# google/uis-rnn

Measured on NVIDIA H100. Metric: predict_frames_per_sec_beam10_256d, higher is better.
Workload: dtype f32

## Files before the change

### uisrnn_b200/csrc/uis_prepass.cuh

```cuda
#pragma once
#include "uis_common.cuh"

namespace uis {

__global__ void cast_f64_f32_kernel(const double* __restrict__ in, float* __restrict__ out, size_t n) {
  size_t i = (size_t)blockIdx.x * blockDim.x + threadIdx.x;
  const size_t stride = (size_t)gridDim.x * blockDim.x;
  for (; i < n; i += stride) out[i] = __double2float_rn(in[i]);
}

__global__ void cast_pad_f64_f32_kernel(const double* __restrict__ in, float* __restrict__ out, size_t rows, int d, int dp) {
  size_t i = (size_t)blockIdx.x * blockDim.x + threadIdx.x;
  const size_t stride = (size_t)gridDim.x * blockDim.x, n = rows * (size_t)dp;
  for (; i < n; i += stride) {
    const size_t r = i / dp;
    const int c = (int)(i % dp);
    out[i] = c < d ? __double2float_rn(in[r * d + c]) : 0.f;
  }
}
__global__ void pad_rows_f32_kernel(const float* __restrict__ in, float* __restrict__ out, size_t rows, int d, int dp) {
  size_t i = (size_t)blockIdx.x * blockDim.x + threadIdx.x;
  const size_t stride = (size_t)gridDim.x * blockDim.x, n = rows * (size_t)dp;
  for (; i < n; i += stride) {
    const size_t r = i / dp;
    const int c = (int)(i % dp);
    out[i] = c < d ? in[r * d + c] : 0.f;
  }
}

constexpr int PBM = 128, PBN = 128, PBK = 16;
__global__ void __launch_bounds__(256) input_proj_kernel(const float* __restrict__ A, const float* __restrict__ Bt,
                                                         const float* __restrict__ bias, float* __restrict__ C,
                                                         int M, int N, int K) {
  __shared__ __align__(16) float As[PBK][PBM + 4];
  __shared__ __align__(16) float Bs[PBK][PBN];
  const int tid = threadIdx.x;
  const int m0 = blockIdx.y * PBM, n0 = blockIdx.x * PBN;
  const int tx = tid % 16, ty = tid / 16;
  float acc[8][8];
#pragma unroll
  for (int i = 0; i < 8; ++i)
#pragma unroll
    for (int q = 0; q < 8; ++q) acc[i][q] = 0.f;

  for (int k0 = 0; k0 < K; k0 += PBK) {
#pragma unroll
    for (int r = 0; r < 2; ++r) {
      const int f = tid + r * 256;
      const int row = f / 4, kq = (f % 4) * 4;
      float4 v = make_float4(0.f, 0.f, 0.f, 0.f);
      if (m0 + row < M && k0 + kq < K) v = *reinterpret_cast<const float4*>(A + (size_t)(m0 + row) * K + k0 + kq);
      As[kq + 0][row] = v.x; As[kq + 1][row] = v.y; As[kq + 2][row] = v.z; As[kq + 3][row] = v.w;
    }
#pragma unroll
    for (int r = 0; r < 2; ++r) {
      const int f = tid + r * 256;
      const int kk = f / 32, nq = (f % 32) * 4;
      float4 v = make_float4(0.f, 0.f, 0.f, 0.f);
      if (k0 + kk < K && n0 + nq < N) v = *reinterpret_cast<const float4*>(Bt + (size_t)(k0 + kk) * N + n0 + nq);
      *reinterpret_cast<float4*>(&Bs[kk][nq]) = v;
    }
    __syncthreads();
#pragma unroll
    for (int kk = 0; kk < PBK; ++kk) {
      const float4 a0 = *reinterpret_cast<const float4*>(&As[kk][ty * 8]);
      const float4 a1 = *reinterpret_cast<const float4*>(&As[kk][ty * 8 + 4]);
      const float4 b0 = *reinterpret_cast<const float4*>(&Bs[kk][tx * 4]);
      const float4 b1 = *reinterpret_cast<const float4*>(&Bs[kk][64 + tx * 4]);
      const float a[8] = {a0.x, a0.y, a0.z, a0.w, a1.x, a1.y, a1.z, a1.w};
      const float b[8] = {b0.x, b0.y, b0.z, b0.w, b1.x, b1.y, b1.z, b1.w};
#pragma unroll
      for (int i = 0; i < 8; ++i)
#pragma unroll
        for (int q = 0; q < 8; ++q) acc[i][q] = fmaf(a[i], b[q], acc[i][q]);
    }
    __syncthreads();
  }
#pragma unroll
  for (int i = 0; i < 8; ++i) {
    const int row = m0 + ty * 8 + i;
    if (row >= M) continue;
#pragma unroll
    for (int h = 0; h < 2; ++h) {
      const int coln = n0 + h * 64 + tx * 4;
      if (coln < N) {
        const float4 bv = *reinterpret_cast<const float4*>(bias + coln);
        float4 o;
        o.x = __fadd_rn(acc[i][h * 4 + 0], bv.x); o.y = __fadd_rn(acc[i][h * 4 + 1], bv.y);
        o.z = __fadd_rn(acc[i][h * 4 + 2], bv.z); o.w = __fadd_rn(acc[i][h * 4 + 3], bv.w);
        *reinterpret_cast<float4*>(C + (size_t)row * N + coln) = o;
      }
    }
  }
}

__global__ void __launch_bounds__(1024) init_state_kernel(const float* __restrict__ whh_t, const float* __restrict__ wih_up_t,
                                  const float* __restrict__ w1_t, const float* __restrict__ w2_t,
                                  const float* __restrict__ bih, const float* __restrict__ bhh,
                                  const float* __restrict__ b1, const float* __restrict__ b2,
                                  const float* __restrict__ h0, int H, int D, int depth, float* __restrict__ mean0,
                                  float* __restrict__ hidden0) {
  extern __shared__ float sm[];
  float* shp = sm; float* shx = sm + H; float* sa = sm + 2 * H;
  const int j = threadIdx.x;
  for (int l = 0; l < depth; ++l) {
    if (j < H) shp[j] = h0[(size_t)l * H + j];
    __syncthreads();
    float hn = 0.f;
    if (j < H) {
      const float* wh = whh_t + (size_t)l * H * 3 * H;
      float ar = 0.f, az = 0.f, an = 0.f;
      for (int k = 0; k < H; ++k) {
        const float x = shp[k];
        ar = fmaf(wh[(size_t)k * 3 * H + j], x, ar);
        az = fmaf(wh[(size_t)k * 3 * H + H + j], x, az);
        an = fmaf(wh[(size_t)k * 3 * H + 2 * H + j], x, an);
      }
      float ir = 0.f, iz = 0.f, in = 0.f;
      if (l > 0) {
        const float* wi = wih_up_t + (size_t)(l - 1) * H * 3 * H;
        for (int k = 0; k < H; ++k) {
          const float x = shx[k];
          ir = fmaf(wi[(size_t)k * 3 * H + j], x, ir);
          iz = fmaf(wi[(size_t)k * 3 * H + H + j], x, iz);
          in = fmaf(wi[(size_t)k * 3 * H + 2 * H + j], x, in);
        }
      }
      const float* bi = bih + (size_t)l * 3 * H;
      const float* bh = bhh + (size_t)l * 3 * H;
      const float r = sigmoid_f32(__fadd_rn(__fadd_rn(ir, bi[j]), __fadd_rn(ar, bh[j])));
      const float z = sigmoid_f32(__fadd_rn(__fadd_rn(iz, bi[H + j]), __fadd_rn(az, bh[H + j])));
      const float n = tanhf(__fadd_rn(__fadd_rn(in, bi[2 * H + j]), __fmul_rn(r, __fadd_rn(an, bh[2 * H + j]))));
      hn = __fadd_rn(__fmul_rn(__fsub_rn(shp[j], n), z), n);
      hidden0[(size_t)l * H + j] = hn;
    }
    __syncthreads();
    if (j < H) shx[j] = hn;
    __syncthreads();
  }
  if (j < H) {
    float a = 0.f;
    for (int k = 0; k < H; ++k) a = fmaf(w1_t[(size_t)k * H + j], shx[k], a);
    sa[j] = fmaxf(__fadd_rn(a, b1[j]), 0.f);
  }
  __syncthreads();
  if (j < D) {
    float a = 0.f;
    for (int k = 0; k < H; ++k) a = fmaf(w2_t[(size_t)k * D + j], sa[k], a);
    mean0[j] = __fadd_rn(a, b2[j]);
  }
}

}
```

### uisrnn_b200/csrc/uis_beam.cuh

```cuda
#pragma once
#include "uis_common.cuh"
#include "uis_beam_tc.cuh"
#include "uis_beam_stat.cuh"

namespace uis {

constexpr int kStages = 2;
constexpr int kStageBytes = 48 * 1024;
constexpr int kInitSlot = 0;
#ifndef UIS_CP_BEAM
#define UIS_CP_BEAM 20
#endif
constexpr int kCPBeam = UIS_CP_BEAM;
template <int H> struct BeamCP { static constexpr int value = H > 512 ? 8 : kCPBeam; };
template <int H> __host__ __device__ constexpr int beam_cp() { return BeamCP<H>::value; }
constexpr int kCPCluster = 12;
constexpr int kXchVals = 24;
constexpr int kCPTree = 16;
template <int H> struct TreeCP { static constexpr int value = H > 512 ? 8 : kCPTree; };
template <int H> __host__ __device__ constexpr int tree_cp() { return TreeCP<H>::value; }
constexpr int kMaxLanes = 8;
constexpr int kMaxBeam = 128;
constexpr int kMaxDepth = 4;

// ... 575 lines not shown
            pool_hidden_cta[(size_t)cc.lane[m0 + m] * lane_pool_h + (size_t)cc.dst[m0 + m] * DH + (size_t)l * H + j] = hnew;
        }
      }
    }
    named_bar_sync(1, NT);
#pragma unroll
    for (int u = 0; u < UPT; ++u)
#pragma unroll
      for (int c = 0; c < NC; ++c)
        reinterpret_cast<float4*>(XB + (size_t)(tid + NT * u) * C::CP)[c] =
            make_float4(hn_out[u][4 * c], hn_out[u][4 * c + 1], hn_out[u][4 * c + 2], hn_out[u][4 * c + 3]);
  }
  named_bar_sync(1, NT);
  if (tid == 0) { const long long now_ = clock64(); ph[2] += now_ - tmark; tmark = now_; }
  {
    float acc[C::R1][4 * NC];
    lin_pass<C, H, C::KT_1, C::KG1, C::R1, NC, true, XCL>(ring, full, empty, it, XB, acc, tid, lane, xrank, xsize);
    float out[UPT][4 * NC];
    ksplit_reduce<C, H, C::KG1, C::R1, UPT, NC>(acc, XA, out, tid);
    if constexpr (XCL) {
      static_assert(UPT * 4 * NC <= kXchVals, "cluster mode: W1 exchange in one round");
      float v[UPT * 4 * NC];
#pragma unroll
      for (int u = 0; u < UPT; ++u)
#pragma unroll
        for (int m = 0; m < 4 * NC; ++m) v[u * 4 * NC + m] = out[u][m];
      xch_allreduce<NT, UPT * 4 * NC>(*xc, v, tid);
#pragma unroll
      for (int u = 0; u < UPT; ++u)
#pragma unroll
        for (int m = 0; m < 4 * NC; ++m) out[u][m] = v[u * 4 * NC + m];
    }
#pragma unroll
    for (int u = 0; u < UPT; ++u)
#pragma unroll
      for (int c = 0; c < NC; ++c) {
        float4 v;
        v.x = fmaxf(__fadd_rn(out[u][4 * c + 0], b1r[u]), 0.f); v.y = fmaxf(__fadd_rn(out[u][4 * c + 1], b1r[u]), 0.f);
        v.z = fmaxf(__fadd_rn(out[u][4 * c + 2], b1r[u]), 0.f); v.w = fmaxf(__fadd_rn(out[u][4 * c + 3], b1r[u]), 0.f);
        reinterpret_cast<float4*>(XA + (size_t)(tid + NT * u) * C::CP)[c] = v;
      }
  }
  named_bar_sync(1, NT);
  if (tid == 0) { const long long now_ = clock64(); ph[3] += now_ - tmark; tmark = now_; }
  {
    float mu_old[4 * NC];
#pragma unroll
    for (int m = 0; m < 4 * NC; ++m)
      mu_old[m] = (m < Mp && tid < D)
                      ? pool_mean_cta[(size_t)cc.lane[m0 + m] * lane_pool_m + (size_t)cc.src[m0 + m] * D + tid]
                      : 0.f;
    float acc[C::R2][4 * NC];
    lin_pass<C, D, C::KT_2, C::KG2, C::R2, NC, true, XCL>(ring, full, empty, it, XA, acc, tid, lane, xrank, xsize);
    float out[1][4 * NC];
    ksplit_reduce<C, D, C::KG2, C::R2, 1, NC>(acc, XA, out, tid);
    if constexpr (XCL) xch_allreduce<NT, 4 * NC>(*xc, out[0], tid);
    if (tid < D) {
#pragma unroll
      for (int m = 0; m < 4 * NC; ++m) {
        if (m < Mp) {
          const float mval = __fadd_rn(out[0][m], b2r);
          const int n = cc.vis[m0 + m];
          const float mu = (n == 0) ? mval
                                    : __fdiv_rn(__fadd_rn(__fmul_rn(mu_old[m], (float)(n - 1)), mval), (float)n);
          pool_mean_cta[(size_t)cc.lane[m0 + m] * lane_pool_m + (size_t)cc.dst[m0 + m] * D + tid] = mu;
        }
      }
    }
  }
}

template <class C, bool DEEP, bool XCL = false>
__device__ __forceinline__ void run_pass_any(const BeamParams& p, const float* ring, uint64_t* full, uint64_t* empty,
                                             unsigned& it, float* XA, float* XB, const ColCtx cc, int m0, int Mp,
                                             float* pool_mean_cta, float* pool_hidden_cta, const float (&bh)[C::RG],
                                             const float (&b1r)[C::UPT], float b2r, int tid, int lane, long long* ph,
                                             long long& tmark, XchCtx* xc = nullptr) {
  const int nc = (Mp + 3) / 4;
#define UIS_RP(NCV, DEEPV) \
  run_pass<C, NCV, DEEPV, XCL>(p, ring, full, empty, it, XA, XB, cc, m0, Mp, pool_mean_cta, pool_hidden_cta, bh, b1r, b2r, tid, lane, ph, tmark, xc)
  if (nc == 1) UIS_RP(1, DEEP); else if (nc == 2) UIS_RP(2, DEEP); else if (nc == 3 || C::CP < 16) UIS_RP(3, DEEP);
  else if (nc == 4 || C::CP < 20) { if constexpr (C::CP >= 16) UIS_RP(4, DEEP); }
  else { if constexpr (C::CP >= 20) UIS_RP(5, DEEP); }
#undef UIS_RP
}

template <int H, int D, int CP, int NT>
__device__ __forceinline__ void stat_pass(const BeamParams& p, const float* sW, float* XA, float* XB, const ColCtx cc, int m0,
                                          int Mp, float* pool_mean_g, float* pool_hidden_g, float* scratch_g, unsigned* bar,
                                          unsigned& epoch, int q, int tid, long long* ph, long long& tmark) {
  using S = StatCfg<H, D>;
  const size_t lane_pool_h = (size_t)p.P * H, lane_pool_m = (size_t)p.P * D;
  stat_dot<H, S::R0, CP, NT>(sW, S::LD, 0, XA, XB, Mp, tid);
  named_bar_sync(1, NT);
  if (tid < S::UG * CP) {
    const int m = tid % CP, u = tid / CP, j = q * S::UG + u;
    if (m < Mp) {
      const float ar = stat_sum<S::R0, CP, NT>(XB, 0 * S::UG + u, m);
      const float az = stat_sum<S::R0, CP, NT>(XB, 1 * S::UG + u, m);
      const float an = stat_sum<S::R0, CP, NT>(XB, 2 * S::UG + u, m);
      const float* gi = p.gi + (size_t)cc.girow[m0 + m] * 3 * H;
      const float r = sigmoid_f32(__fadd_rn(gi[j], __fadd_rn(ar, __ldg(p.bhh + j))));
      const float z = sigmoid_f32(__fadd_rn(gi[H + j], __fadd_rn(az, __ldg(p.bhh + H + j))));
      const float n = tanhf(__fadd_rn(gi[2 * H + j], __fmul_rn(r, __fadd_rn(an, __ldg(p.bhh + 2 * H + j)))));
      const float ho = XA[(size_t)j * CP + m];
      pool_hidden_g[(size_t)cc.lane[m0 + m] * lane_pool_h + (size_t)cc.dst[m0 + m] * H + j] =
          __fadd_rn(__fmul_rn(__fsub_rn(ho, n), z), n);
    }
  }
  stat_group_sync<NT>(bar, epoch, tid);
  if (tid == 0) { const long long now_ = clock64(); ph[2] += now_ - tmark; tmark = now_; }
  for (int i = tid; i < Mp * H; i += NT) {
    const int m = i / H, k = i % H;
    XA[(size_t)k * CP + m] = __ldcg(pool_hidden_g + (size_t)cc.lane[m0 + m] * lane_pool_h + (size_t)cc.dst[m0 + m] * H + k);
  }
  named_bar_sync(1, NT);
  stat_dot<H, S::R1, CP, NT>(sW, S::LD, S::R0, XA, XB, Mp, tid);
  named_bar_sync(1, NT);
  if (tid < S::R1 * CP) {
    const int m = tid % CP, u = tid / CP, j = q * S::R1 + u;
    if (m < Mp)
      scratch_g[(size_t)m * H + j] = fmaxf(__fadd_rn(stat_sum<S::R1, CP, NT>(XB, u, m), __ldg(p.b1 + j)), 0.f);
  }
  stat_group_sync<NT>(bar, epoch, tid);
  if (tid == 0) { const long long now_ = clock64(); ph[3] += now_ - tmark; tmark = now_; }
  for (int i = tid; i < Mp * H; i += NT) {
    const int m = i / H, k = i % H;
    XA[(size_t)k * CP + m] = __ldcg(scratch_g + (size_t)m * H + k);
  }
  named_bar_sync(1, NT);
  stat_dot<H, S::R2, CP, NT>(sW, S::LD, S::R0 + S::R1, XA, XB, Mp, tid);
  named_bar_sync(1, NT);
  if (tid < S::R2 * CP) {
    const int m = tid % CP, u = tid / CP, d = q * S::R2 + u;
    if (m < Mp) {
      const float mval = __fadd_rn(stat_sum<S::R2, CP, NT>(XB, u, m), __ldg(p.b2 + d));
      const int n = cc.vis[m0 + m];
      const float mu_old = __ldcg(pool_mean_g + (size_t)cc.lane[m0 + m] * lane_pool_m + (size_t)cc.src[m0 + m] * D + d);
      const float mu = (n == 0) ? mval : __fdiv_rn(__fadd_rn(__fmul_rn(mu_old, (float)(n - 1)), mval), (float)n);
      pool_mean_g[(size_t)cc.lane[m0 + m] * lane_pool_m + (size_t)cc.dst[m0 + m] * D + d] = mu;
    }
  }
  stat_group_sync<NT>(bar, epoch, tid);
}

template <int H, int D, int N, class Idle>
__device__ __forceinline__ void tc_run_pass(const BeamParams& p, const unsigned char* ring, unsigned char* bop,
                                            const TcBars& tb, unsigned& tbox, const ColCtx cc, int m0, int Mp,
                                            float* pool_mean_cta, float* pool_hidden_cta, float* scratch_cta, int tid,
                                            int lane, int warp, long long* ph, long long& tmark, long long* tstat,
                                            Idle idle_work) {
  using TC = TcCfg<H, D, N>;
  constexpr int NT = 256, NI = N / 8;
  constexpr int KB = (NI == 6) ? 2 : 4, WB = (NI == 6) ? 3 : NI;
  auto hslot = [&](int g, int s) { return pool_hidden_cta + (size_t)(g * p.P + s) * H; };
  auto mslot = [&](int g, int s) { return pool_mean_cta + (size_t)(g * p.P + s) * D; };
  const int wg = warp >> 2;
  const int r0 = wg * 64 + (warp & 3) * 16 + (lane >> 2);
  const int cq = 2 * (lane & 3);
  long long* ts = (tid == 0) ? tstat : nullptr;
  const long long t_in = clock64();
  float acc[TC::NACC];
  auto stage_b = [&](auto src, float scale) {
    const long long w0 = clock64();
    tc_gather_b<H, N, NT>(bop, src, Mp, scale, tid);
    tc_publish_b<NT>();
    if (ts) ts[2] += clock64() - w0;
  };
  if (tid < Mp && (tid == 0 || cc.lane[m0 + tid] != cc.lane[m0 + tid - 1]))
    prefetch_l2_bulk(p.gi + (size_t)cc.girow[m0 + tid] * 3 * H, 3 * H * 4);
  stage_b([&](int m) -> const float* {
    return hslot(cc.lane[m0 + m], cc.src[m0 + m]); }, p.tc_sh);
  if (tid == 0) { const long long now_ = clock64(); ph[1] += now_ - tmark; tmark = now_; }
  idle_work();
  if (tid == 0) { const long long now_ = clock64(); ph[7] += now_ - tmark; tmark = now_; }
  static_assert(H >= NT, "gate parking: 2 * (N / 2) * NT floats within the [N][H] scratch");
  float* park = scratch_cta + tid;
  for (int ut = 0; ut < TC::UT; ++ut) {
    const int j0 = ut * 128 + r0;
    {
      float v[TC::NV];
#pragma unroll
      for (int g = 0; g < 2; ++g) {
        tc_tile<TC>(acc, ring, bop, tb, tbox, wg, lane, ts);
        tc_fold<TC>(acc, v, p.tc_inv_hh);
        const float bh[2] = {__ldg(p.bhh + g * H + j0), __ldg(p.bhh + g * H + j0 + 8)};
#pragma unroll
        for (int q = 0; q < TC::NV; ++q) park[(g * TC::NV + q) * NT] = __fadd_rn(v[q], bh[(q >> 1) & 1]);
      }
    }
    tc_tile<TC>(acc, ring, bop, tb, tbox, wg, lane, ts);
    float an[TC::NV];
    tc_fold<TC>(acc, an, p.tc_inv_hh);
    {
      const float bh[2] = {__ldg(p.bhh + 2 * H + j0), __ldg(p.bhh + 2 * H + j0 + 8)};
#pragma unroll
      for (int q = 0; q < TC::NV; ++q) an[q] = __fadd_rn(an[q], bh[(q >> 1) & 1]);
    }
#pragma unroll
    for (int k0 = 0; k0 < 2 * NI; k0 += KB) {
      float gr[KB][2], gz[KB][2], gn[KB][2], pr[KB][2], pz[KB][2], ho[KB][2];
#pragma unroll
      for (int b = 0; b < KB; ++b) {
        const int i = (k0 + b) >> 1, e = (k0 + b) & 1, m = 8 * i + cq + e;
        if (m < Mp) {
          const float* gi = p.gi + (size_t)cc.girow[m0 + m] * 3 * H + j0;
          const float* hs = hslot(cc.lane[m0 + m], cc.src[m0 + m]) + j0;
#pragma unroll
          for (int h = 0; h < 2; ++h) {
            const int v = 4 * i + 2 * h + e;
            gr[b][h] = __ldg(gi + 8 * h); gz[b][h] = __ldg(gi + H + 8 * h); gn[b][h] = __ldg(gi + 2 * H + 8 * h);
            pr[b][h] = park[v * NT]; pz[b][h] = park[(TC::NV + v) * NT];
            ho[b][h] = hs[8 * h];
          }
        }
      }
#pragma unroll
      for (int b = 0; b < KB; ++b) {
        const int i = (k0 + b) >> 1, e = (k0 + b) & 1, m = 8 * i + cq + e;
        if (m < Mp) {
          float* hd = hslot(cc.lane[m0 + m], cc.dst[m0 + m]) + j0;
#pragma unroll
          for (int h = 0; h < 2; ++h) {
            const int v = 4 * i + 2 * h + e;
            const float rg = sigmoid_f32(__fadd_rn(gr[b][h], pr[b][h]));
            const float zg = sigmoid_f32(__fadd_rn(gz[b][h], pz[b][h]));
            const float ng = tanhf(__fadd_rn(gn[b][h], __fmul_rn(rg, an[v])));
            hd[8 * h] = __fadd_rn(__fmul_rn(__fsub_rn(ho[b][h], ng), zg), ng);
          }
        }
      }
    }
  }
  named_bar_sync(1, NT);
  if (tid == 0) { const long long now_ = clock64(); ph[2] += now_ - tmark; tmark = now_; }
  stage_b([&](int m) -> const float* {
    return hslot(cc.lane[m0 + m], cc.dst[m0 + m]); }, p.tc_sh);
  for (int mt = 0; mt < TC::T2; ++mt) {
    float v1[TC::NV];
    tc_tile<TC>(acc, ring, bop, tb, tbox, wg, lane, ts);
    tc_fold<TC>(acc, v1, p.tc_inv_1);
#pragma unroll
    for (int h = 0; h < 2; ++h) {
      const int j = mt * 128 + r0 + 8 * h;
      const float b1j = __ldg(p.b1 + j);
#pragma unroll
      for (int i = 0; i < NI; ++i)
#pragma unroll
        for (int e = 0; e < 2; ++e) {
          const int m = 8 * i + cq + e;
          if (m < Mp) scratch_cta[(size_t)m * H + j] = fmaxf(__fadd_rn(v1[4 * i + 2 * h + e], b1j), 0.f);
        }
    }
  }
  named_bar_sync(1, NT);
  if (tid == 0) { const long long now_ = clock64(); ph[3] += now_ - tmark; tmark = now_; }
  stage_b([&](int m) -> const float* { return scratch_cta + (size_t)m * H; }, p.tc_sa);
  for (int mt = 0; mt < TC::T3; ++mt) {
    float v2[TC::NV];
    tc_tile<TC>(acc, ring, bop, tb, tbox, wg, lane, ts);
    tc_fold<TC>(acc, v2, p.tc_inv_2);
#pragma unroll
    for (int h = 0; h < 2; ++h) {
      const int d = mt * 128 + r0 + 8 * h;
      const float b2d = __ldg(p.b2 + d);
#pragma unroll
      for (int i0 = 0; i0 < NI; i0 += WB) {
        float mu_old[WB][2];
#pragma unroll
        for (int b = 0; b < WB; ++b)
#pragma unroll
          for (int e = 0; e < 2; ++e) {
            const int m = 8 * (i0 + b) + cq + e;
            if (m < Mp) mu_old[b][e] = mslot(cc.lane[m0 + m], cc.src[m0 + m])[d];
          }
#pragma unroll
        for (int b = 0; b < WB; ++b)
#pragma unroll
          for (int e = 0; e < 2; ++e) {
            const int m = 8 * (i0 + b) + cq + e;
            if (m < Mp) {
              const float mval = __fadd_rn(v2[4 * (i0 + b) + 2 * h + e], b2d);
              const int n = cc.vis[m0 + m];
              const float mu = (n == 0) ? mval : __fdiv_rn(__fadd_rn(__fmul_rn(mu_old[b][e], (float)(n - 1)), mval), (float)n);
              mslot(cc.lane[m0 + m], cc.dst[m0 + m])[d] = mu;
            }
          }
      }
    }
  }
  if (ts) ts[3] += clock64() - t_in;
}

template <int H, int D, bool DEEP, int XM = 0, int TCN = 0>
__global__ void __launch_bounds__(Cfg<H, D>::BLOCK, 1) uis_beam_kernel(const __grid_constant__ BeamParams p) {
  constexpr bool XCL = XM == 1, STAT = XM == 2;
  using C = Cfg<H, D, (XCL || STAT) ? kCPCluster : BeamCP<H>::value>;
  constexpr int NT = C::NT, NW = C::NW, UPT = C::UPT;
  constexpr bool TC = TCN > 0;
  static_assert(!TC || (!DEEP && !XCL && !STAT && NT == 256 && C::REBALANCE), "tensor-core pass: depth 1, one CTA per lane group");
  static_assert(!STAT || (!DEEP && NT == 256), "stationary-weights mode: depth 1, 256 consumer threads");
  using TCC = TcCfg<TC ? H : 512, TC ? D : 256, TC ? TCN : 48>;
  extern __shared__ __align__(128) unsigned char smem_raw[];
  unsigned char* smem = TC ? reinterpret_cast<unsigned char*>((reinterpret_cast<uintptr_t>(smem_raw) + 1023) & ~(uintptr_t)1023)
                           : smem_raw;
  const int B = p.B, Kcap = p.Kcap, G = p.G;
  const SmemLayout L_ = make_layout<H, D, C::CP, XCL, TCN, STAT>(B, Kcap, G);
  const SmemLayout& L = TC ? p.tc_layout : L_;
  if constexpr (TC)
    if (p.tc_layout.total == 0) __trap();
  const int sq = STAT ? (int)(blockIdx.x % kStatGroup) : 0, sgroup = STAT ? (int)(blockIdx.x / kStatGroup) : 0;
  float* ring = reinterpret_cast<float*>(smem + L.ring);
  float* XA = reinterpret_cast<float*>(smem + L.xa);
  float* XB = reinterpret_cast<float*>(smem + L.xb);
  float* wv = reinterpret_cast<float*>(smem + L.wv);
  int* colarr = reinterpret_cast<int*>(smem + L.cols);
  uint64_t* full = reinterpret_cast<uint64_t*>(smem + L.bars);
  uint64_t* empty = full + (TC ? TCC::STAGES : kStages);
  volatile int* misc = reinterpret_cast<volatile int*>(smem + L.misc);
  TcBars tb{full, empty};

  const int tid = threadIdx.x, lane = tid & 31, warp = tid >> 5;

  if (tid == 0) {
    if constexpr (TC) {
      for (int s = 0; s < TCC::STAGES; ++s) {
        mbar_init(&tb.full[s], 1);
        mbar_init(&tb.empty[s], NW);
      }
    } else {
      for (int s = 0; s < kStages; ++s) {
        mbar_init(&full[s], 1);
        mbar_init(&empty[s], NW);
      }
    }
    for (int i = 0; i < 16; ++i) misc[i] = 0;
    if constexpr (TC)
      for (int i = 16; i < 20; ++i) reinterpret_cast<long long*>(smem + L.phase)[i] = 0;
    if constexpr (XCL) {
      uint64_t* xbar = reinterpret_cast<uint64_t*>(smem + L.xbar);
      mbar_init(&xbar[0], cluster_nctarank() - 1);
      mbar_init(&xbar[1], cluster_nctarank() - 1);
      misc[MI_QNEXT] = (int)cluster_id_x();
    }
    if constexpr (STAT) misc[MI_QNEXT] = sgroup;
    fence_mbar_init();
  }
  __syncthreads();
  if constexpr (XCL) cluster_sync_all();

  if (warp >= NW) {
    if constexpr (STAT) return;
    if constexpr (TC) asm volatile("setmaxnreg.dec.sync.aligned.u32 40;");
    else if constexpr (C::REBALANCE) asm volatile("setmaxnreg.dec.sync.aligned.u32 24;");
    if constexpr (TC) {
      if (warp == NW) tc_producer_loop<TCC, H>(&p.tc_wmap, reinterpret_cast<unsigned char*>(ring), tb, &misc[MI_DONE]);
    } else {
      if (warp == NW && lane == 0) producer_loop<C, XCL>(p, ring, full, empty, misc);
    }
    return;
  }
  if constexpr (TC) asm volatile("setmaxnreg.inc.sync.aligned.u32 232;");
  else if constexpr (C::REBALANCE && !STAT) asm volatile("setmaxnreg.inc.sync.aligned.u32 240;");

  auto lane_base = [&](int g) -> unsigned char* { return smem + L.lanes + (size_t)g * L.lane_stride; };
  auto LSp = [&](int g) -> volatile int* { return reinterpret_cast<volatile int*>(lane_base(g) + L.l_ls); };
  const int DH = p.depth * H;
  const size_t pool_m_stride = (size_t)p.P * D, pool_h_stride = (size_t)p.P * DH;
  float* pool_mean_cta = p.pool_mean + (size_t)(STAT ? sgroup : blockIdx.x) * G * pool_m_stride;
  float* pool_hidden_cta = p.pool_hidden + (size_t)(STAT ? sgroup : blockIdx.x) * G * pool_h_stride;
  unsigned* bp_cta = p.bp + (size_t)blockIdx.x * G * p.maxN * B;
  const unsigned PW = (unsigned)(p.P + 31) / 32;
  const float INF = __int_as_float(0x7f800000);
  const int bbits = B > 32 ? 7 : 5;

  float bh[C::RG], b1r[UPT];
#pragma unroll
  for (int i = 0; i < C::RG; ++i) bh[i] = TC ? 0.f : p.bhh[(i / UPT) * H + tid + NT * (i % UPT)];
#pragma unroll
  for (int u = 0; u < UPT; ++u) b1r[u] = TC ? 0.f : p.b1[tid + NT * u];
  const float b2r = (tid < D && !TC) ? p.b2[tid] : 0.f;
// ... 617 lines not shown
```

### uisrnn_b200/csrc/uis_beam_tc.cuh

```cuda
#pragma once
#include <cuda.h>
#include <cuda_fp16.h>
#include "uis_common.cuh"

namespace uis {

constexpr int kTcBoxBytes = 16384;

template <int H, int D, int N>
struct TcCfg {
  static constexpr int KA = H / 64;
  static constexpr int UT = H / 128;
  static constexpr int T1 = 3 * UT, T2 = H / 128, T3 = D / 128;
  static constexpr int TILES = T1 + T2 + T3;
  static constexpr int ROWS = 3 * H + H + D;
  static constexpr int NP = 2 * N;
  static constexpr int NACC = NP / 2;
  static constexpr int NV = N / 2;
  static constexpr int ATOM_BYTES = NP * 128;
  static constexpr int BOP_BYTES = KA * ATOM_BYTES;
  static constexpr int STAGES = (N <= 32) ? 8 : 4;
  static_assert(H % 128 == 0 && D % 128 == 0, "tensor-core pass: 128-row tiles");
  static_assert(NP == 64 || NP == 96, "wgmma instantiations: N = 32 or 48 columns");
};

__device__ __forceinline__ uint64_t tc_desc_sw128(uint32_t saddr) {
  uint64_t d = 0;
  d |= (uint64_t)((saddr >> 4) & 0x3fff);
  d |= (uint64_t)1 << 16;
  d |= (uint64_t)(1024 >> 4) << 32;
  d |= (uint64_t)1 << 62;
  return d;
}
__device__ __forceinline__ void wgmma_fence() { asm volatile("wgmma.fence.sync.aligned;" ::: "memory"); }
__device__ __forceinline__ void wgmma_commit() { asm volatile("wgmma.commit_group.sync.aligned;" ::: "memory"); }
template <int PENDING>
__device__ __forceinline__ void wgmma_wait() { asm volatile("wgmma.wait_group.sync.aligned %0;" ::"n"(PENDING) : "memory"); }

template <int NP> struct Wgmma;
template <> struct Wgmma<96> {
  static __device__ __forceinline__ void mma(float (&d)[48], uint64_t adesc, uint64_t bdesc, uint32_t acc) {
    asm volatile(
        "{\n\t.reg .pred p;\n\tsetp.ne.b32 p, %50, 0;\n\t"
        "wgmma.mma_async.sync.aligned.m64n96k16.f32.f16.f16 {%0, %1, %2, %3, %4, %5, %6, %7, %8, %9, %10, %11, %12, %13, %14, %15, %16, %17, %18, %19, %20, %21, %22, %23, %24, %25, %26, %27, %28, %29, %30, %31, %32, %33, %34, %35, %36, %37, %38, %39, %40, %41, %42, %43, %44, %45, %46, %47}, %48, %49, p, 1, 1, 0, 0;\n\t}"
        : "+f"(d[0]), "+f"(d[1]), "+f"(d[2]), "+f"(d[3]), "+f"(d[4]), "+f"(d[5]), "+f"(d[6]), "+f"(d[7]), "+f"(d[8]), "+f"(d[9]), "+f"(d[10]), "+f"(d[11]), "+f"(d[12]), "+f"(d[13]), "+f"(d[14]), "+f"(d[15]), "+f"(d[16]), "+f"(d[17]), "+f"(d[18]), "+f"(d[19]), "+f"(d[20]), "+f"(d[21]), "+f"(d[22]), "+f"(d[23]), "+f"(d[24]), "+f"(d[25]), "+f"(d[26]), "+f"(d[27]), "+f"(d[28]), "+f"(d[29]), "+f"(d[30]), "+f"(d[31]), "+f"(d[32]), "+f"(d[33]), "+f"(d[34]), "+f"(d[35]), "+f"(d[36]), "+f"(d[37]), "+f"(d[38]), "+f"(d[39]), "+f"(d[40]), "+f"(d[41]), "+f"(d[42]), "+f"(d[43]), "+f"(d[44]), "+f"(d[45]), "+f"(d[46]), "+f"(d[47])
        : "l"(adesc), "l"(bdesc), "r"(acc)
        : "memory");
  }
};
template <> struct Wgmma<64> {
  static __device__ __forceinline__ void mma(float (&d)[32], uint64_t adesc, uint64_t bdesc, uint32_t acc) {
    asm volatile(
        "{\n\t.reg .pred p;\n\tsetp.ne.b32 p, %34, 0;\n\t"
        "wgmma.mma_async.sync.aligned.m64n64k16.f32.f16.f16 {%0, %1, %2, %3, %4, %5, %6, %7, %8, %9, %10, %11, %12, %13, %14, %15, %16, %17, %18, %19, %20, %21, %22, %23, %24, %25, %26, %27, %28, %29, %30, %31}, %32, %33, p, 1, 1, 0, 0;\n\t}"
        : "+f"(d[0]), "+f"(d[1]), "+f"(d[2]), "+f"(d[3]), "+f"(d[4]), "+f"(d[5]), "+f"(d[6]), "+f"(d[7]), "+f"(d[8]), "+f"(d[9]), "+f"(d[10]), "+f"(d[11]), "+f"(d[12]), "+f"(d[13]), "+f"(d[14]), "+f"(d[15]), "+f"(d[16]), "+f"(d[17]), "+f"(d[18]), "+f"(d[19]), "+f"(d[20]), "+f"(d[21]), "+f"(d[22]), "+f"(d[23]), "+f"(d[24]), "+f"(d[25]), "+f"(d[26]), "+f"(d[27]), "+f"(d[28]), "+f"(d[29]), "+f"(d[30]), "+f"(d[31])
        : "l"(adesc), "l"(bdesc), "r"(acc)
        : "memory");
  }
};

__device__ __forceinline__ void tc_tma_load_2d(void* dst, const CUtensorMap* map, int c0, int c1, uint64_t* bar) {
  asm volatile(
      "cp.async.bulk.tensor.2d.shared::cluster.global.mbarrier::complete_tx::bytes [%0], [%1, {%3, %4}], [%2];" ::"r"(
          smem_u32(dst)),
      "l"(reinterpret_cast<uint64_t>(map)), "r"(smem_u32(bar)), "r"(c0), "r"(c1)
      : "memory");
}

__device__ __forceinline__ void tc_mbar_wait(uint64_t* bar, uint32_t parity) {
  if (mbar_try_wait(bar, parity)) return;
  const long long t0 = clock64();
  unsigned spins = 0;
  while (!mbar_try_wait(bar, parity)) {
    if ((++spins & 0x3ffu) == 0 && clock64() - t0 > 8000000000ll) __trap();
  }
}

__device__ __forceinline__ bool tc_wait_or_done(uint64_t* bar, uint32_t parity, volatile int* done_flag) {
  for (;;) {
    uint32_t ok;
    asm volatile(
        "{\n\t.reg .pred p;\n\t"
        "mbarrier.try_wait.parity.shared::cta.b64 p, [%1], %2, %3;\n\t"
        "selp.u32 %0, 1, 0, p;\n\t}"
        : "=r"(ok)
        : "r"(smem_u32(bar)), "r"(parity), "r"(4000u)
        : "memory");
    if (ok) return true;
    if (*done_flag) return false;
  }
}

__device__ __forceinline__ bool tc_elect_one() {
  uint32_t pred;
  asm volatile("{\n\t.reg .pred p;\n\telect.sync _|p, 0xffffffff;\n\tselp.u32 %0, 1, 0, p;\n\t}" : "=r"(pred));
  return pred != 0;
}

struct TcBars {
  uint64_t* full;
  uint64_t* empty;
};

template <class TC, int H>
__device__ __forceinline__ int tc_tile_row0(int t) {
  if (t < TC::T1) return (t % 3) * H + (t / 3) * 128;
  return 3 * H + (t - TC::T1) * 128;
}

template <class TC, int H>
__device__ void tc_producer_loop(const CUtensorMap* wmap, unsigned char* ring, const TcBars& b, volatile int* done_flag) {
  unsigned it = 0;
  bool run = true;
  while (run) {
    for (int t = 0; t < TC::TILES && run; ++t) {
      const int row0 = tc_tile_row0<TC, H>(t);
      for (int pl = 0; pl < 2 && run; ++pl) {
        for (int ka = 0; ka < TC::KA; ++ka, ++it) {
          const unsigned s = it % TC::STAGES, ph = (it / TC::STAGES) & 1;
          if (!tc_wait_or_done(&b.empty[s], ph ^ 1, done_flag)) { run = false; break; }
          if (tc_elect_one()) {
            mbar_arrive_expect_tx(&b.full[s], kTcBoxBytes);
            tc_tma_load_2d(ring + (size_t)s * kTcBoxBytes, wmap, ka * 64, pl * TC::ROWS + row0, &b.full[s]);
          }
          __syncwarp();
        }
      }
    }
  }
  for (unsigned j = (it > (unsigned)TC::STAGES) ? it - TC::STAGES : 0; j < it; ++j)
    tc_mbar_wait(&b.full[j % TC::STAGES], (j / TC::STAGES) & 1);
}

template <class TC>
__device__ __forceinline__ void tc_tile(float (&acc)[TC::NACC], const unsigned char* ring, const unsigned char* bop,
                                        const TcBars& b, unsigned& box, int wg, int lane, long long* tstat) {
  const uint64_t desc0 = tc_desc_sw128(0);
  const uint32_t a16 = (smem_u32(ring) + (uint32_t)wg * (kTcBoxBytes / 2)) >> 4, b16 = smem_u32(bop) >> 4;
#pragma unroll
  for (int i = 0; i < TC::NACC; ++i) acc[i] = 0.f;
  unsigned prev = 0;
#pragma unroll 1
  for (int q = 0; q < 2 * TC::KA; ++q, ++box) {
    const unsigned s = box % TC::STAGES, par = (box / TC::STAGES) & 1u;
    if (!mbar_try_wait(&b.full[s], par)) {
      const long long w0 = tstat ? clock64() : 0;
      tc_mbar_wait(&b.full[s], par);
      if (tstat) tstat[0] += clock64() - w0;
    }
    const uint64_t adesc = desc0 + (uint64_t)(a16 + s * (kTcBoxBytes >> 4));
    const uint64_t bdesc = desc0 + (uint64_t)(b16 + (uint32_t)(q % TC::KA) * (TC::ATOM_BYTES >> 4));
    wgmma_fence();
#pragma unroll
    for (int kk = 0; kk < 4; ++kk) Wgmma<TC::NP>::mma(acc, adesc + 2 * kk, bdesc + 2 * kk, (q | kk) != 0);
    wgmma_commit();
    if (q > 0) {
      wgmma_wait<1>();
      __syncwarp();
      if (lane == 0) mbar_arrive(&b.empty[prev]);
    }
    prev = s;
  }
  const long long w0 = tstat ? clock64() : 0;
  wgmma_wait<0>();
  if (tstat) tstat[1] += clock64() - w0;
  __syncwarp();
  if (lane == 0) mbar_arrive(&b.empty[prev]);
}

template <class TC>
__device__ __forceinline__ void tc_fold(const float (&acc)[TC::NACC], float (&v)[TC::NV], float inv) {
  constexpr int LO = TC::NACC / 2;
#pragma unroll
  for (int i = 0; i < TC::NV; ++i) v[i] = __fmul_rn(__fmaf_rn(acc[LO + i], 0x1p-11f, acc[i]), inv);
}

template <int H, int N, int NTHREADS, class SrcFn>
__device__ __forceinline__ void tc_gather_b(unsigned char* bop, SrcFn src, int Mp, float scale, int tid) {
  constexpr int PPC = H / 2;
  constexpr int CG = NTHREADS / PPC;
  static_assert(NTHREADS % PPC == 0 && CG >= 1, "gather mapping");
  const int pair = tid % PPC, cg = tid / PPC;
  const int k = 2 * pair;
  const uint32_t koff = (uint32_t)(k >> 6) * (2u * N * 128u) + (uint32_t)(k & 7) * 2u;
  const uint32_t kchunk = (uint32_t)(k & 63) >> 3;
  constexpr int UNR = 8;
  for (int m0 = cg; m0 < Mp; m0 += CG * UNR) {
    float2 v[UNR];
#pragma unroll
    for (int u = 0; u < UNR; ++u) {
      const int m = m0 + u * CG;
      v[u] = (m < Mp) ? *reinterpret_cast<const float2*>(src(m) + k) : make_float2(0.f, 0.f);
    }
#pragma unroll
    for (int u = 0; u < UNR; ++u) {
      const int m = m0 + u * CG;
      if (m < Mp) {
        const float x0 = v[u].x * scale, x1 = v[u].y * scale;
        const __half h0 = __float2half_rn(x0), h1 = __float2half_rn(x1);
        const __half l0 = __float2half_rn((x0 - __half2float(h0)) * 2048.f);
        const __half l1 = __float2half_rn((x1 - __half2float(h1)) * 2048.f);
        const uint32_t off = koff + (uint32_t)m * 128u + ((kchunk ^ ((uint32_t)m & 7u)) << 4);
        *reinterpret_cast<__half2*>(bop + off) = __halves2half2(h0, h1);
        *reinterpret_cast<__half2*>(bop + off + (uint32_t)N * 128u) = __halves2half2(l0, l1);
      }
    }
  }
}
template <int NTHREADS>
__device__ __forceinline__ void tc_publish_b() {
  fence_proxy_async();
  named_bar_sync(1, NTHREADS);
}

}
```

Measured before the change: 2.175 million.

## Double-buffer input projection GEMM tiles with cp.async prefetch

Converts the input projection GEMM to double-buffered shared memory. The next K-tile of A goes through registers and the next tile of B is fetched with cp.async, both overlapped with the FMA loop on the current tile. This removes one __syncthreads per iteration and hides global load latency. It also adds launch_bounds minBlocks=2, which caps registers and doubles shared memory use and could cause spills. The input projection is a prepass, so its share of end-to-end beam-search frames/sec is likely small.

New measurement: 2.190 million (median of 6 runs). No clear change (+0.7%).

```diff
diff --git a/uisrnn_b200/csrc/uis_prepass.cuh b/uisrnn_b200/csrc/uis_prepass.cuh
--- a/uisrnn_b200/csrc/uis_prepass.cuh
+++ b/uisrnn_b200/csrc/uis_prepass.cuh
@@ -29,44 +29,57 @@
 }
 
 constexpr int PBM = 128, PBN = 128, PBK = 16;
-__global__ void __launch_bounds__(256) input_proj_kernel(const float* __restrict__ A, const float* __restrict__ Bt,
-                                                         const float* __restrict__ bias, float* __restrict__ C,
-                                                         int M, int N, int K) {
-  __shared__ __align__(16) float As[PBK][PBM + 4];
-  __shared__ __align__(16) float Bs[PBK][PBN];
+__global__ void __launch_bounds__(256, 2) input_proj_kernel(const float* __restrict__ A, const float* __restrict__ Bt,
+                                                            const float* __restrict__ bias, float* __restrict__ C,
+                                                            int M, int N, int K) {
+  __shared__ __align__(16) float As[2][PBK][PBM + 4];
+  __shared__ __align__(16) float Bs[2][PBK][PBN];
   const int tid = threadIdx.x;
   const int m0 = blockIdx.y * PBM, n0 = blockIdx.x * PBN;
   const int tx = tid % 16, ty = tid / 16;
+  float4 ra[2];
+  auto load = [&](int k0, int s) {
+#pragma unroll
+    for (int r = 0; r < 2; ++r) {
+      const int f = tid + r * 256;
+      const int row = f / 4, kq = (f % 4) * 4;
+      ra[r] = make_float4(0.f, 0.f, 0.f, 0.f);
+      if (m0 + row < M && k0 + kq < K) ra[r] = *reinterpret_cast<const float4*>(A + (size_t)(m0 + row) * K + k0 + kq);
+      const int kk = f / 32, nq = (f % 32) * 4;
+      float* bs = &Bs[s][kk][nq];
+      if (k0 + kk < K && n0 + nq < N) cp_async16(bs, Bt + (size_t)(k0 + kk) * N + n0 + nq);
+      else *reinterpret_cast<float4*>(bs) = make_float4(0.f, 0.f, 0.f, 0.f);
+    }
+    cp_async_commit();
+  };
+  auto store = [&](int s) {
+#pragma unroll
+    for (int r = 0; r < 2; ++r) {
+      const int f = tid + r * 256;
+      const int row = f / 4, kq = (f % 4) * 4;
+      As[s][kq + 0][row] = ra[r].x; As[s][kq + 1][row] = ra[r].y; As[s][kq + 2][row] = ra[r].z; As[s][kq + 3][row] = ra[r].w;
+    }
+    cp_async_wait_all();
+  };
   float acc[8][8];
 #pragma unroll
   for (int i = 0; i < 8; ++i)
 #pragma unroll
     for (int q = 0; q < 8; ++q) acc[i][q] = 0.f;
 
+  load(0, 0);
+  store(0);
+  __syncthreads();
+  int s = 0;
   for (int k0 = 0; k0 < K; k0 += PBK) {
-#pragma unroll
-    for (int r = 0; r < 2; ++r) {
-      const int f = tid + r * 256;
-      const int row = f / 4, kq = (f % 4) * 4;
-      float4 v = make_float4(0.f, 0.f, 0.f, 0.f);
-      if (m0 + row < M && k0 + kq < K) v = *reinterpret_cast<const float4*>(A + (size_t)(m0 + row) * K + k0 + kq);
-      As[kq + 0][row] = v.x; As[kq + 1][row] = v.y; As[kq + 2][row] = v.z; As[kq + 3][row] = v.w;
-    }
-#pragma unroll
-    for (int r = 0; r < 2; ++r) {
-      const int f = tid + r * 256;
-      const int kk = f / 32, nq = (f % 32) * 4;
-      float4 v = make_float4(0.f, 0.f, 0.f, 0.f);
-      if (k0 + kk < K && n0 + nq < N) v = *reinterpret_cast<const float4*>(Bt + (size_t)(k0 + kk) * N + n0 + nq);
-      *reinterpret_cast<float4*>(&Bs[kk][nq]) = v;
-    }
-    __syncthreads();
+    const bool more = k0 + PBK < K;
+    if (more) load(k0 + PBK, s ^ 1);
 #pragma unroll
     for (int kk = 0; kk < PBK; ++kk) {
-      const float4 a0 = *reinterpret_cast<const float4*>(&As[kk][ty * 8]);
-      const float4 a1 = *reinterpret_cast<const float4*>(&As[kk][ty * 8 + 4]);
-      const float4 b0 = *reinterpret_cast<const float4*>(&Bs[kk][tx * 4]);
-      const float4 b1 = *reinterpret_cast<const float4*>(&Bs[kk][64 + tx * 4]);
+      const float4 a0 = *reinterpret_cast<const float4*>(&As[s][kk][ty * 8]);
+      const float4 a1 = *reinterpret_cast<const float4*>(&As[s][kk][ty * 8 + 4]);
+      const float4 b0 = *reinterpret_cast<const float4*>(&Bs[s][kk][tx * 4]);
+      const float4 b1 = *reinterpret_cast<const float4*>(&Bs[s][kk][64 + tx * 4]);
       const float a[8] = {a0.x, a0.y, a0.z, a0.w, a1.x, a1.y, a1.z, a1.w};
       const float b[8] = {b0.x, b0.y, b0.z, b0.w, b1.x, b1.y, b1.z, b1.w};
 #pragma unroll
@@ -74,7 +87,9 @@
 #pragma unroll
         for (int q = 0; q < 8; ++q) acc[i][q] = fmaf(a[i], b[q], acc[i][q]);
     }
+    if (more) store(s ^ 1);
     __syncthreads();
+    s ^= 1;
   }
 #pragma unroll
   for (int i = 0; i < 8; ++i) {
```

## Reorder GRU gate tiles so gates are consumed in registers, not parked in smem

Applied to the files above, without the earlier changes.

The weight-tile stream for the GRU pass changes order to new, reset, then update. The reset gate is consumed right after its tile is folded to produce the candidate state, and the update gate is applied straight from registers in a second sweep. This removes the shared-memory parking of the r/z gate pre-activations, with its stores and reloads, and the batch size KB is fixed at 4. In exchange the gate loop is split into two passes, register pressure rises, and producer and consumer must agree on the new tile ordering.

Measured after the change: 2.197 million before, 2.236 million after (median of 6 runs). 1.8% higher.

```diff
diff --git a/uisrnn_b200/csrc/uis_beam.cuh b/uisrnn_b200/csrc/uis_beam.cuh
--- a/uisrnn_b200/csrc/uis_beam.cuh
+++ b/uisrnn_b200/csrc/uis_beam.cuh
@@ -751,7 +751,7 @@
                                             Idle idle_work) {
   using TC = TcCfg<H, D, N>;
   constexpr int NT = 256, NI = N / 8;
-  constexpr int KB = (NI == 6) ? 2 : 4, WB = (NI == 6) ? 3 : NI;
+  constexpr int KB = 4, WB = (NI == 6) ? 3 : NI;
   auto hslot = [&](int g, int s) { return pool_hidden_cta + (size_t)(g * p.P + s) * H; };
   auto mslot = [&](int g, int s) { return pool_mean_cta + (size_t)(g * p.P + s) * D; };
   const int wg = warp >> 2;
@@ -773,32 +773,52 @@
   if (tid == 0) { const long long now_ = clock64(); ph[1] += now_ - tmark; tmark = now_; }
   idle_work();
   if (tid == 0) { const long long now_ = clock64(); ph[7] += now_ - tmark; tmark = now_; }
-  static_assert(H >= NT, "gate parking: 2 * (N / 2) * NT floats within the [N][H] scratch");
-  float* park = scratch_cta + tid;
+  auto gate_bias = [&](int g, int j0, float (&bh)[2]) {
+    bh[0] = __ldg(p.bhh + g * H + j0);
+    bh[1] = __ldg(p.bhh + g * H + j0 + 8);
+  };
   for (int ut = 0; ut < TC::UT; ++ut) {
     const int j0 = ut * 128 + r0;
-    {
-      float v[TC::NV];
-#pragma unroll
-      for (int g = 0; g < 2; ++g) {
-        tc_tile<TC>(acc, ring, bop, tb, tbox, wg, lane, ts);
-        tc_fold<TC>(acc, v, p.tc_inv_hh);
-        const float bh[2] = {__ldg(p.bhh + g * H + j0), __ldg(p.bhh + g * H + j0 + 8)};
-#pragma unroll
-        for (int q = 0; q < TC::NV; ++q) park[(g * TC::NV + q) * NT] = __fadd_rn(v[q], bh[(q >> 1) & 1]);
-      }
-    }
+    float an[TC::NV], v[TC::NV], bh[2];
     tc_tile<TC>(acc, ring, bop, tb, tbox, wg, lane, ts);
-    float an[TC::NV];
     tc_fold<TC>(acc, an, p.tc_inv_hh);
-    {
-      const float bh[2] = {__ldg(p.bhh + 2 * H + j0), __ldg(p.bhh + 2 * H + j0 + 8)};
-#pragma unroll
-      for (int q = 0; q < TC::NV; ++q) an[q] = __fadd_rn(an[q], bh[(q >> 1) & 1]);
-    }
+    gate_bias(2, j0, bh);
+#pragma unroll
+    for (int q = 0; q < TC::NV; ++q) an[q] = __fadd_rn(an[q], bh[(q >> 1) & 1]);
+    tc_tile<TC>(acc, ring, bop, tb, tbox, wg, lane, ts);
+    tc_fold<TC>(acc, v, p.tc_inv_hh);
+    gate_bias(0, j0, bh);
 #pragma unroll
     for (int k0 = 0; k0 < 2 * NI; k0 += KB) {
-      float gr[KB][2], gz[KB][2], gn[KB][2], pr[KB][2], pz[KB][2], ho[KB][2];
+      float gr[KB][2], gn[KB][2];
+#pragma unroll
+      for (int b = 0; b < KB; ++b) {
+        const int i = (k0 + b) >> 1, e = (k0 + b) & 1, m = 8 * i + cq + e;
+        if (m < Mp) {
+          const float* gi = p.gi + (size_t)cc.girow[m0 + m] * 3 * H + j0;
+#pragma unroll
+          for (int h = 0; h < 2; ++h) { gr[b][h] = __ldg(gi + 8 * h); gn[b][h] = __ldg(gi + 2 * H + 8 * h); }
+        }
+      }
+#pragma unroll
+      for (int b = 0; b < KB; ++b) {
+        const int i = (k0 + b) >> 1, e = (k0 + b) & 1, m = 8 * i + cq + e;
+        if (m < Mp) {
+#pragma unroll
+          for (int h = 0; h < 2; ++h) {
+            const int q = 4 * i + 2 * h + e;
+            const float rg = sigmoid_f32(__fadd_rn(gr[b][h], __fadd_rn(v[q], bh[h])));
+            an[q] = tanhf(__fadd_rn(gn[b][h], __fmul_rn(rg, an[q])));
+          }
+        }
+      }
+    }
+    tc_tile<TC>(acc, ring, bop, tb, tbox, wg, lane, ts);
+    tc_fold<TC>(acc, v, p.tc_inv_hh);
+    gate_bias(1, j0, bh);
+#pragma unroll
+    for (int k0 = 0; k0 < 2 * NI; k0 += KB) {
+      float gz[KB][2], ho[KB][2];
 #pragma unroll
       for (int b = 0; b < KB; ++b) {
         const int i = (k0 + b) >> 1, e = (k0 + b) & 1, m = 8 * i + cq + e;
@@ -806,12 +826,7 @@
           const float* gi = p.gi + (size_t)cc.girow[m0 + m] * 3 * H + j0;
           const float* hs = hslot(cc.lane[m0 + m], cc.src[m0 + m]) + j0;
 #pragma unroll
-          for (int h = 0; h < 2; ++h) {
-            const int v = 4 * i + 2 * h + e;
-            gr[b][h] = __ldg(gi + 8 * h); gz[b][h] = __ldg(gi + H + 8 * h); gn[b][h] = __ldg(gi + 2 * H + 8 * h);
-            pr[b][h] = park[v * NT]; pz[b][h] = park[(TC::NV + v) * NT];
-            ho[b][h] = hs[8 * h];
-          }
+          for (int h = 0; h < 2; ++h) { gz[b][h] = __ldg(gi + H + 8 * h); ho[b][h] = hs[8 * h]; }
         }
       }
 #pragma unroll
@@ -821,11 +836,9 @@
           float* hd = hslot(cc.lane[m0 + m], cc.dst[m0 + m]) + j0;
 #pragma unroll
           for (int h = 0; h < 2; ++h) {
-            const int v = 4 * i + 2 * h + e;
-            const float rg = sigmoid_f32(__fadd_rn(gr[b][h], pr[b][h]));
-            const float zg = sigmoid_f32(__fadd_rn(gz[b][h], pz[b][h]));
-            const float ng = tanhf(__fadd_rn(gn[b][h], __fmul_rn(rg, an[v])));
-            hd[8 * h] = __fadd_rn(__fmul_rn(__fsub_rn(ho[b][h], ng), zg), ng);
+            const int q = 4 * i + 2 * h + e;
+            const float zg = sigmoid_f32(__fadd_rn(gz[b][h], __fadd_rn(v[q], bh[h])));
+            hd[8 * h] = __fadd_rn(__fmul_rn(__fsub_rn(ho[b][h], an[q]), zg), an[q]);
           }
         }
       }
diff --git a/uisrnn_b200/csrc/uis_beam_tc.cuh b/uisrnn_b200/csrc/uis_beam_tc.cuh
--- a/uisrnn_b200/csrc/uis_beam_tc.cuh
+++ b/uisrnn_b200/csrc/uis_beam_tc.cuh
@@ -104,7 +104,7 @@
 
 template <class TC, int H>
 __device__ __forceinline__ int tc_tile_row0(int t) {
-  if (t < TC::T1) return (t % 3) * H + (t / 3) * 128;
+  if (t < TC::T1) return ((t + 2) % 3) * H + (t / 3) * 128;
   return 3 * H + (t - TC::T1) * 128;
 }
 
```
